# xiaohong-huang/RTK-Visual-Inertial-Navigation

Measured on AMD Instinct MI355X. Metric: gauss_newton_iterations_per_sec, higher is better.
Workload: dtype f64; 1 GPU; BASELINE cfg4: batch of 512 independent cfg3 windows (20 keyframes, 300 features, 3000 observations, 19 IMU factors, 10 satellites x 20 epochs carrier-phase+pseudorange, gauge prior) over the job, 8 dogleg iterations per solve; windows=512, windows_rank0=512

## Files before the change

### rtk_visual_inertial_navigation_amd/csrc/swf_dev.h

```cpp
#pragma once
#include <hip/hip_runtime.h>
#include <stdint.h>
#include "../../include/swf_types.h"

#define SWF_WAVE 64

struct WinRec {
    int x_base, x_n;
    int blk_base, n_blk;
    int loc_base, n_loc, n_e, n_red;
    long long S_base;
    long long Lt_base;
    int proj0, proj1;
    int lm0, lm1;
    int fr_base, nF;
    long long P_base;
    int gf0, gf1;
    int cl0, cl1;
    int pair0, pair1;
    int fsb0, fsb1;
    int tail_dim;
    int n_pose_blk;
    int lmb0, lmb1;
    int pch0, pch1;
// ... 36 lines not shown
    int j_off, r_off;
    int pad0, pad1;
};

struct Pair {
    int win;
    int ra, rb, la, lb;
    int fa, fb;
    int c0, c1;
    int is_diag;
    int loc_a;
    int fsb0, fsb1;
    int n, m;
    long long S_base, P_base;
    long long q_base;
};

struct AsmWin {
    int se0, ne;
    int ve0, nv;
    int n_red, m;
    int loc_base;
    int fs_base;
    int v_base;
    int win;
    long long C_base, S_base, P_base, q_base;
};
#define AS_NC(c) ((c) & 4095u)
#define AS_NP(c) (((c) >> 12) & 31u)
#define AS_NH(c) (((c) >> 17) & 4095u)
#define AS_DIAG(c) (((c) >> 29) & 1u)
#define AS_SOLD(c) (((c) >> 30) & 1u)

struct DevBatch {
    int n_win;
    int n_x, n_loc_total;
    int max_iter_trace;
    double* x; double* xc; double* x0;
    double* g; double* diag; double* rhs; double* y; double* step;
    double* vc;
    double* S; double* L;
    double* Wk;
    double* Linv;
    const WinRec* win; WinState* ws; swf_iteration* trace;
    const int* blk_xoff; const int* blk_loc; const int* blk_gs;
    const int* loc2x;
    const unsigned char* x_var;
    int n_proj;
    const int* p_win; const int* p_xpose; const int* p_xex; const int* p_xlm;
    const int* p_lpose; const int* p_llm; const int* p_fr; const int* p_lm;
    const double* p_uv;
    double* p_r; double* p_Jp; double* p_Jl;
    double* p_cpart; double* p_apart;
    int n_fsb; const int* fsb_win; const int* fsb_obs0; const int* fsb_perm; const int* fsb_foff; const int* fsb_foff0; const int* fsb_out0;
    double* fs_part;
    double* jsc;
    int n_lm;
    const int* lm_win; const int* lm_obs0; const int* lm_loc; const int* lm_col;
    double* lm_Einv; double* lm_g;
    double* P;
    double* lmq;
    const int* lmb_rec; int n_lmb;
    const int* sch_c0; const int* sch_rec;
    const int* sch_km;
    const unsigned long long* lm_fmask;
    int n_fr;
    const int* fr_obs0; const int* fr_obs;
    const int* fr_red;
    int n_gf;
    const GFac* gf;
    const int* s_x; const int* s_loc; const int* s_ls; const int* s_joff; const int* s_ccol;
    double* g_r; double* g_J; double* g_cost; double* g_aux;
    const double* imu_pre; const double* cp_dat; const double* pr_dat; const double* dop_dat; const double* sp_w;
    const double* gx_dat;
    int n_imu; const int* imu_gf;
    int n_idp; const int* idp_gf;
    int n_sc;  const int* sc_gf;
    int n_prior; const int* prior_gf;
    int n_pch; const int* pch_q; const int* pch_r0; const int* prior_nch;
    double* pr_cpart; double* pr_apart;
    const int* prior_dim; const long long* prior_Joff; const int* prior_roff; const int* prior_x0off;
    const double* prior_J; const double* prior_r0; const double* prior_x0;
    const double* prior_Jt;
    const int* prior_colloc;
    const int* prior_colcc;
    const int* s_pcol; const int* s_pxo;
    int n_cl;
    const Clique* cl;
    const int* cl_fac; const int* cl_frow;
    const int* cm_loc; const int* cm_ls; const int* cm_col;
    double* C; double* cv_graw; double* cv_dgraw; double* cv_cs; double* cE;
    const int* cv_loc;
    int n_clc[5]; const Clique* clc_rec[5];
    int n_cle; const Clique* cle_rec;
    int n_pair;
    const long long* pc_coff; const int* pc_cld; const int* pc_voff;
    int n_pd, n_po; const Pair* pair_d; const Pair* pair_o;
    const AsmWin* asw; int as_max_ne, as_max_nv;
    const int* as_dst; const unsigned* as_cnt; const int* as_src0; const int* as_aux; const int* as_src;
    const int* av_loc; const int* av_red; const unsigned* av_cnt; const int* av_src0; const int* av_i; const int* av_src;
    const unsigned* s_tnz;
    int spec;
    int rr_nmax;
};

__device__ __forceinline__ void qmul(const double* a, const double* b, double* o) {
    double ax = a[0], ay = a[1], az = a[2], aw = a[3];
// ... 247 lines not shown
```

### rtk_visual_inertial_navigation_amd/csrc/swf_engine.hip

```cpp
#include <hip/hip_runtime.h>
#include <algorithm>
#include <array>
#include <chrono>
#include <cmath>
#include <cstdio>
#include <cstdlib>
#include <cstring>
#include <map>
#include <string>
#include <memory>
#include <thread>
#include <vector>
#include "../../include/swf_solver.h"
#include "swf_kernels2.h"
#include "swf_kernels3.h"
#include "swf_kernels4.h"
#include "swf_lambda.h"

static thread_local std::string g_err;
static int fail(int code, const std::string& msg) { g_err = msg; return code; }
#define HIPCHK(x) do { hipError_t e_ = (x); if (e_ != hipSuccess) return fail(SWF_E_NODEVICE, std::string(#x) + ": " + hipGetErrorString(e_)); } while (0)

extern "C" const char* swf_last_error(void) { return g_err.c_str(); }
void swf_internal_set_error(const std::string& m) { g_err = m; }
// ... 868 lines not shown
                if (B.lm_loc[l] < 0) continue;
                int k = B.lm_obs0[l + 1] - B.lm_obs0[l];
                if (k > 64) { P.release(); delete b; return fail(SWF_E_UNSUPPORTED, "landmark with more than 64 observations"); }
                trs[(size_t)(l - W.lm0)] = tile_rows(B.lm_fmask[l]);
                ord.push_back(l);
            }
            auto key = [&](int l) { unsigned t = trs[(size_t)(l - W.lm0)]; int lo = t ? __builtin_ctz(t) : 0, hi = t ? 31 - __builtin_clz(t) : 0; return hi * 64 + lo; };
            std::stable_sort(ord.begin(), ord.end(), [&](int x, int y) { return key(x) < key(y); });
            const int first_task = (int)(rec.size() / 32);
            task_tiles.clear();
            size_t at = 0; int lw = 4;
            auto new_task = [&]() { at = rec.size(); rec.resize(at + 32, 0); for (int g = 0; g < 4; g++) rec[at + g * 8] = -1; task_tiles.emplace_back((size_t)ntl, 0u); lw = 0; };
            for (int l : ord) {
                int o0 = B.lm_obs0[l], k = B.lm_obs0[l + 1] - o0;
                if (lw >= 4) new_task();
                int* r = &rec[at + (size_t)lw * 8];
                r[0] = l; r[1] = B.lm_loc[l]; r[2] = o0; r[3] = o0 + k; r[4] = 3 * lw; r[5] = 0; r[6] = 0; r[7] = 0;
                unsigned t = trs[(size_t)(l - W.lm0)];
                const unsigned ks = lw == 0 ? 1u : lw == 1 ? 3u : lw == 2 ? 6u : 4u;
                std::vector<unsigned>& tt = task_tiles.back();
                for (int tr = 0; tr < nt; tr++) {
                    if (!((t >> tr) & 1u)) continue;
                    tt[(size_t)tr] |= ks;
                    for (int tc = 0; tc < tr; tc++) if ((t >> tc) & 1u) tt[(size_t)(nt + tr * (tr - 1) / 2 + tc)] |= ks;
                }
                lw++;
            }
            if (task_tiles.size() & 1) new_task();
            const int ntask = (int)task_tiles.size();
            for (int c = 0; c < ntask / TW; c++) {
                size_t kw = km.size(); km.resize(kw + (size_t)b->ls_kms, 0);
                for (int g = 0; g < TW; g++) {
                    const std::vector<unsigned>& tt = task_tiles[(size_t)(c * TW + g)];
                    for (int e = 0; e < ntl; e++) if (tt[(size_t)e]) {
                        b->lm_schur_mfma += __builtin_popcount(tt[(size_t)e]);
                        int lp = e / (NCW * TPW), r = e % (NCW * TPW), sl = r / NCW, cw = r % NCW;
                        km[kw + (size_t)(lp * NCW + cw)] |= (tt[(size_t)e] << (3 * g)) << (3 * TW * sl);
                    }
                }
            }
            const int np = ntask / 2;
            for (int sp = 0; sp < GEMM_SPLIT; sp++) c0.push_back(first_task + 2 * (int)((long long)sp * np / GEMM_SPLIT));
        }
        c0.push_back((int)(rec.size() / 32));
        rec.resize(rec.size() + (size_t)32 * 4 * LS_NB, 0);
        km.resize(km.size() + (size_t)b->ls_kms * 2, 0);
        PUT(sch_c0, c0); PUT(sch_rec, rec); PUT(sch_km, km);
    }
    D.n_fr = B.n_fr;
    B.fr_obs0.push_back((int)B.fr_obs.size());
    PUT(fr_obs0, B.fr_obs0); PUT(fr_obs, B.fr_obs); PUT(fr_red, B.fr_red);
    D.n_fsb = (int)B.fsb_win.size();
    B.fsb_obs0.push_back(D.n_proj); B.fsb_perm.resize((size_t)D.n_proj + 1, 0);
    PUT(fsb_win, B.fsb_win); PUT(fsb_obs0, B.fsb_obs0); PUT(fsb_perm, B.fsb_perm); PUT(fsb_foff, B.fsb_foff); PUT(fsb_foff0, B.fsb_foff0); PUT(fsb_out0, B.fsb_out0);
    rc |= P.zeros((size_t)B.fs_tot * FS_VAL, &D.fs_part);
    rc |= P.zeros((size_t)std::max<long long>(B.n_loc, 1), &D.jsc);
    D.n_gf = (int)B.gf.size();
    PUT(gf, B.gf);
    PUT(s_x, B.s_x); PUT(s_loc, B.s_loc); PUT(s_ls, B.s_ls); PUT(s_joff, B.s_joff); PUT(s_ccol, B.s_ccol);
    PUT(imu_pre, B.imu_pre); PUT(cp_dat, B.cp_dat); PUT(pr_dat, B.pr_dat); PUT(dop_dat, B.dop_dat); PUT(sp_w, B.sp_w); PUT(gx_dat, B.gx_dat);
    D.n_imu = (int)B.imu_gf.size(); D.n_sc = (int)B.sc_gf.size(); D.n_prior = (int)B.prior_gf.size();
    PUT(imu_gf, B.imu_gf); PUT(sc_gf, B.sc_gf); PUT(prior_gf, B.prior_gf); D.n_idp = (int)B.idp_gf.size(); PUT(idp_gf, B.idp_gf);
    PUT(prior_dim, B.prior_dim); PUT(prior_Joff, B.prior_Joff); PUT(prior_roff, B.prior_roff); PUT(prior_x0off, B.prior_x0off);
    {
        std::vector<double> Jt(B.prior_J.size());
        for (size_t k = 0; k < B.prior_dim.size(); k++) {
            const size_t n = (size_t)B.prior_dim[k]; const double* J = B.prior_J.data() + B.prior_Joff[k]; double* T = Jt.data() + B.prior_Joff[k];
            for (size_t r = 0; r < n; r++) for (size_t c = 0; c < n; c++) T[c * n + r] = J[r * n + c];
        }
        PUT(prior_Jt, Jt);
        std::vector<int> cl(B.prior_r0.size(), -1), cc(B.prior_r0.size(), -1), pcol(B.s_ls.size(), 0), pxo(B.s_ls.size(), 0);
        for (const GFac& G : B.gf) {
            if (G.type != GF_PRIOR) continue;
            int col = 0, xo = 0;
            for (int t = 0; t < G.nslot; t++) {
                int l = B.s_ls[G.slot0 + t], lo = B.s_loc[G.slot0 + t], mc = B.s_ccol[G.slot0 + t];
                pcol[G.slot0 + t] = col; pxo[G.slot0 + t] = xo;
                for (int q = 0; q < l; q++) {
                    cl[(size_t)B.prior_roff[G.data] + col + q] = lo >= 0 ? lo + q : -1;
                    cc[(size_t)B.prior_roff[G.data] + col + q] = mc >= 0 ? mc + q : -1;
                }
                col += l; xo += (l == 6 ? 7 : l);
            }
        }
        PUT(prior_colloc, cl); PUT(prior_colcc, cc); PUT(s_pcol, pcol); PUT(s_pxo, pxo);
    }
    PUT(prior_J, B.prior_J); PUT(prior_r0, B.prior_r0); PUT(prior_x0, B.prior_x0);
    D.n_cl = (int)B.cl.size();
    PUT(cl, B.cl); PUT(cl_fac, B.cl_fac); PUT(cl_frow, B.cl_frow); PUT(cm_loc, B.cm_loc); PUT(cm_ls, B.cm_ls); PUT(cm_col, B.cm_col);
    {
        std::vector<int> cvl((size_t)std::max(B.v_tot, 1), 0);
        for (const Clique& c : B.cl)
            for (int m = c.mem0; m < c.mem1; m++)
                for (int q = 0; q < B.cm_ls[(size_t)m]; q++) cvl[(size_t)c.v_off + (size_t)B.cm_col[(size_t)m] + (size_t)q] = B.cm_loc[(size_t)m] + q;
        PUT(cv_loc, cvl);
    }
    D.n_pair = (int)B.pair.size();
    PUT(pc_coff, B.pc_coff); PUT(pc_cld, B.pc_cld); PUT(pc_voff, B.pc_voff);
    {
        std::vector<int> pd, po, clc[5], cle;
        for (size_t i = 0; i < B.pair.size(); i++) {
            Pair& Pq = B.pair[i]; const WinRec& Rw = B.win[Pq.win];
            Pq.fsb0 = Rw.fsb0; Pq.fsb1 = Rw.fsb1; Pq.n = Rw.n_red; Pq.m = 6 * Rw.nF; Pq.S_base = Rw.S_base; Pq.P_base = Rw.P_base; Pq.q_base = (long long)6 * Rw.fr_base * GEMM_SPLIT;
            if (b->s_direct && !Pq.is_diag && Pq.fa >= 0 && Pq.fb >= 0 && Pq.c0 == Pq.c1) continue;
            (Pq.is_diag ? pd : po).push_back((int)i);
        }
        std::stable_sort(po.begin(), po.end(), [&](int a, int c) {
// ... 1118 lines not shown
    if (!ok) return fail(SWF_E_NODEVICE, "download failed");
    return SWF_OK;
}

#ifdef SWF_PROFILE_CHOL
extern "C" int swf_debug_chol_stamps(unsigned long long* out) {
    if (hipDeviceSynchronize() != hipSuccess) return SWF_E_NODEVICE;
    if (hipMemcpyFromSymbol(out, HIP_SYMBOL(g_chol_stamps), 64 * sizeof(unsigned long long)) != hipSuccess) return SWF_E_NODEVICE;
    return SWF_OK;
}
#endif

#ifdef SWF_PROFILE_CHOLW
extern "C" int swf_debug_chol_wstep(int step) {
    if (hipDeviceSynchronize() != hipSuccess) return SWF_E_NODEVICE;
    unsigned long long z[16 * 8] = { 0 };
    if (hipMemcpyToSymbol(HIP_SYMBOL(g_chol_wst), z, sizeof(z)) != hipSuccess) return SWF_E_NODEVICE;
    if (hipMemcpyToSymbol(HIP_SYMBOL(g_chol_wstep), &step, sizeof(int)) != hipSuccess) return SWF_E_NODEVICE;
    return SWF_OK;
}
extern "C" int swf_debug_chol_wstamps(unsigned long long* out) {
    if (hipDeviceSynchronize() != hipSuccess) return SWF_E_NODEVICE;
    if (hipMemcpyFromSymbol(out, HIP_SYMBOL(g_chol_wst), 16 * 8 * sizeof(unsigned long long)) != hipSuccess) return SWF_E_NODEVICE;
    return SWF_OK;
}
extern "C" int swf_debug_chol_pstamps(unsigned long long* out) {
    if (hipDeviceSynchronize() != hipSuccess) return SWF_E_NODEVICE;
    if (hipMemcpyFromSymbol(out, HIP_SYMBOL(g_chol_pst), 16 * sizeof(unsigned long long)) != hipSuccess) return SWF_E_NODEVICE;
    return SWF_OK;
}
extern "C" int swf_debug_chol_cstamps(unsigned long long* out) {
    if (hipDeviceSynchronize() != hipSuccess) return SWF_E_NODEVICE;
    if (hipMemcpyFromSymbol(out, HIP_SYMBOL(g_chol_cst), 32 * sizeof(unsigned long long)) != hipSuccess) return SWF_E_NODEVICE;
    return SWF_OK;
}
#endif

#ifdef SWF_PROFILE_DOG
extern "C" int swf_debug_dog_stamps(unsigned long long* out) {
    if (hipDeviceSynchronize() != hipSuccess) return SWF_E_NODEVICE;
    if (hipMemcpyFromSymbol(out, HIP_SYMBOL(g_dog_stamps), 16 * sizeof(unsigned long long)) != hipSuccess) return SWF_E_NODEVICE;
    return SWF_OK;
}
#endif

#ifdef SWF_PROFILE_CLQ
extern "C" int swf_debug_clq_stamps(unsigned long long* out) {
    if (hipDeviceSynchronize() != hipSuccess) return SWF_E_NODEVICE;
    if (hipMemcpyFromSymbol(out, HIP_SYMBOL(g_clq_stamps), 16 * sizeof(unsigned long long)) != hipSuccess) return SWF_E_NODEVICE;
    return SWF_OK;
}
#endif

#ifdef SWF_PROFILE_GEMM
extern "C" int swf_debug_gemm_stamps(unsigned long long* out) {
    if (hipDeviceSynchronize() != hipSuccess) return SWF_E_NODEVICE;
    if (hipMemcpyFromSymbol(out, HIP_SYMBOL(g_gemm_stamps), 16 * sizeof(unsigned long long)) != hipSuccess) return SWF_E_NODEVICE;
    return SWF_OK;
}
#endif


struct swf_composite {
    CompArgs A{};
    std::vector<void*> bufs;
    int n = 0, nmax = 0, nmin = 0; long long sumM = 0, sumN = 0, sumG = 0, sumG2 = 0;
    std::vector<int> M;
    bool eigen_root = false;
    hipStream_t stream = nullptr;
    ~swf_composite() { for (void* p : bufs) (void)hipFree(p); }
};

extern "C" int swf_composite_destroy(swf_composite* c) { delete c; return SWF_OK; }

extern "C" int swf_composite_create(int32_t n, const int32_t* M, const int32_t* N, const double* pose, const double* sb,
                                    const double* pose_lin, const double* sb_lin, const double* Hpp, const double* HpN,
                                    const double* rhs_p, const double* HNN, const double* rhsN, const double* pre,
                                    const double pbg[3], const double gw[3], void* stream, swf_composite** out) {
    if (!out || n <= 0 || !M || !N || !pose || !sb || !pose_lin || !sb_lin || !Hpp || !HpN || !rhs_p || !HNN || !rhsN || !pre || !pbg || !gw)
        return fail(SWF_E_INVALID, "swf_composite_create: null argument");
    std::vector<int> eo(n + 1, 0), no(n + 1, 0);
    std::vector<long long> pno(n + 1, 0), nno(n + 1, 0), go(n + 1, 0), g2o(n + 1, 0);
    int nmax_ = 0, nmin_ = 1 << 30;
    for (int f = 0; f < n; f++) {
        if (M[f] < 1) return fail(SWF_E_INVALID, "composite factor without hidden epochs");
        if (N[f] < 0 || N[f] > CO_MAXN) return fail(SWF_E_UNSUPPORTED, "composite factor with more than 64 ambiguities");
        nmax_ = std::max(nmax_, (int)N[f]); nmin_ = std::min(nmin_, (int)N[f]);
        eo[f + 1] = eo[f] + M[f]; no[f + 1] = no[f] + N[f];
        pno[f + 1] = pno[f] + 15LL * M[f] * N[f]; nno[f + 1] = nno[f] + (long long)N[f] * N[f];
        go[f + 1] = go[f] + 30 + N[f]; g2o[f + 1] = g2o[f] + (long long)(30 + N[f]) * (30 + N[f]);
    }
    std::unique_ptr<swf_composite> c(new swf_composite());
    c->n = n; c->nmax = nmax_; c->nmin = nmin_; c->sumM = eo[n]; c->sumN = no[n]; c->sumG = go[n]; c->sumG2 = g2o[n]; c->stream = (hipStream_t)stream;
    bool bad = false;
    auto up = [&](const void* src, size_t bytes) -> void* {
        void* d = nullptr;
        if (hipMalloc(&d, std::max<size_t>(bytes, 8)) != hipSuccess) { bad = true; return nullptr; }
        c->bufs.push_back(d);
        if (src) { if (hipMemcpy(d, src, bytes, hipMemcpyHostToDevice) != hipSuccess) bad = true; }
        else if (hipMemset(d, 0, std::max<size_t>(bytes, 8)) != hipSuccess) bad = true;
        return d;
    };
    CompArgs& A = c->A;
    const size_t D = sizeof(double);
    A.n = n;
    A.M = (const int*)up(M, n * sizeof(int)); A.N = (const int*)up(N, n * sizeof(int));
// ... 86 lines not shown
```

### rtk_visual_inertial_navigation_amd/csrc/swf_kernels.h

```cpp
#pragma once
#include "swf_dev.h"

struct DevOpt {
    int max_iter, step_mode, strategy, jacobi;
    double r0, max_r, min_r, min_rel_dec, ftol, gtol, ptol, min_mu, max_mu, mu_inc, min_diag, max_diag;
};



__device__ __forceinline__ double damp_diag(const DevOpt& O, double d, double* jsc_slot, bool first) {
    if (!O.jacobi) return clampd(d, O.min_diag, O.max_diag);
    double q;
    if (first) { double r = 1.0 + sqrt(d > 0.0 ? d : 0.0); q = r * r; *jsc_slot = q; }
    else q = *jsc_slot;
    return clampd(d / q, O.min_diag, O.max_diag) * q;
}

template <bool JAC> __device__ __forceinline__ bool eval_gate(const DevBatch& B, const WinState& s) { return B.spec == 2 ? true : (JAC && !B.spec) ? s.need_lin != 0 : s.eval_cand != 0; }
template <bool JAC> __device__ __forceinline__ const double* eval_src(const DevBatch& B) { return (JAC && !B.spec) ? B.x : B.xc; }

#define CLIGHT_D 299792458.0
#define OMGE_D 7.2921151467E-5

template <bool JAC, bool STORE>
__device__ __forceinline__ double proj_core(const DevBatch& B, int i, const WinRec& W, const double* P, const double* E, const double* X,
                                          double u0, double u1, bool jp, bool jl, double* keep);
template <bool JAC, bool STORE = true>
__device__ __forceinline__ double d_eval_proj_at(const DevBatch& B, int i, double* keep) {
    int w = B.p_win[i];
    const WinState& s = B.ws[w];
    if (!eval_gate<JAC>(B, s)) return 0.0;
    const WinRec& W = B.win[w];
    const double* xs = eval_src<JAC>(B);
    const double* pose = xs + B.p_xpose[i];
    const double* ex = xs + B.p_xex[i];
    const double* lm = xs + B.p_xlm[i];
    double P[7], E[7], X[3];
#pragma unroll
    for (int k = 0; k < 7; k++) { P[k] = pose[k]; E[k] = ex[k]; }
    X[0] = lm[0]; X[1] = lm[1]; X[2] = lm[2];
    return proj_core<JAC, STORE>(B, i, W, P, E, X, B.p_uv[2 * i], B.p_uv[2 * i + 1], JAC && B.p_lpose[i] >= 0, JAC && B.p_llm[i] >= 0, keep);
}
template <bool JAC, bool STORE>
__device__ __forceinline__ double proj_core(const DevBatch& B, int i, const WinRec& W, const double* P, const double* E, const double* X,
                                          double u0, double u1, bool jp, bool jl, double* keep) {
    double Qj_inv[4], qic_inv[4], d[3], pts_imu[3], t[3], pc[3];
    qinv(P + 3, Qj_inv);
    qinv(E + 3, qic_inv);
    d[0] = X[0] - P[0]; d[1] = X[1] - P[1]; d[2] = X[2] - P[2];
    qrot(Qj_inv, d, pts_imu);
    t[0] = pts_imu[0] + W.pbg[0] - E[0]; t[1] = pts_imu[1] + W.pbg[1] - E[1]; t[2] = pts_imu[2] + W.pbg[2] - E[2];
    qrot(qic_inv, t, pc);
    double dep = pc[2], si = W.proj_sqrt_info;
    double r0 = si * (pc[0] / dep - u0);
    double r1 = si * (pc[1] / dep - u1);
    double sr = 1.0, cost;
    double sq = r0 * r0 + r1 * r1;
    if (W.proj_loss_a > 0) {
        double b = W.proj_loss_a * W.proj_loss_a, c = 1.0 / b;
        double sum = 1.0 + sq * c, inv = 1.0 / sum;
        cost = 0.5 * b * log(sum);
        sr = sqrt(inv > 2.2250738585072014e-308 ? inv : 2.2250738585072014e-308);
    } else cost = 0.5 * sq;
    if (!JAC) return cost;
    int n = B.n_proj;
    if (STORE) { B.p_r[i] = r0 * sr; B.p_r[n + i] = r1 * sr; }
    if (keep) { keep[12] = r0 * sr; keep[13] = r1 * sr; }
    if (!jp && !jl) return cost;
    double Rj[9], ric[9], ricT[9], RjT[9], A[9];
    q2R(P + 3, Rj); q2R(E + 3, ric);
    mat3T(ric, ricT); mat3T(Rj, RjT);
    double red[6] = { si * (1. / dep), 0, si * (-pc[0] / (dep * dep)), 0, si * (1. / dep), si * (-pc[1] / (dep * dep)) };
    mat3mul(ricT, RjT, A);
    if (jp) {
        double S[9], Bm[9];
        skew3(pts_imu, S);
        mat3mul(ricT, S, Bm);
#pragma unroll
        for (int a = 0; a < 2; a++)
#pragma unroll
            for (int j = 0; j < 3; j++) {
                double u = 0, v = 0;
#pragma unroll
                for (int k = 0; k < 3; k++) { u += red[a * 3 + k] * -A[k * 3 + j]; v += red[a * 3 + k] * Bm[k * 3 + j]; }
                if (STORE) { if (!jl) B.p_Jp[(a * 6 + j) * n + i] = u * sr; B.p_Jp[(a * 6 + 3 + j) * n + i] = v * sr; }
                if (keep) { keep[a * 6 + j] = u * sr; keep[a * 6 + 3 + j] = v * sr; }
            }
    }
    if (jl) {
#pragma unroll
        for (int a = 0; a < 2; a++)
#pragma unroll
            for (int j = 0; j < 3; j++) {
                double u = 0;
#pragma unroll
                for (int k = 0; k < 3; k++) u += red[a * 3 + k] * A[k * 3 + j];
                if (STORE) B.p_Jl[(a * 3 + j) * n + i] = u * sr;
                if (keep) keep[14 + a * 3 + j] = u * sr;
            }
    }
    return cost;
}

__device__ __forceinline__ void d_eval_proj_cost(const DevBatch& B, int blk) {
    __shared__ double csum[16];
    const int w = B.fsb_win[blk];
    if (!eval_gate<false>(B, B.ws[w])) return;
    const int o_beg = B.fsb_obs0[blk], cnt = B.fsb_obs0[blk + 1] - o_beg, tid = threadIdx.x;
    double c = 0.0;
    if (tid < cnt) c = d_eval_proj_at<false>(B, o_beg + tid, nullptr);
    c = block_sum(c, csum);
    if (tid == 0) B.p_cpart[blk] = c;
}

__device__ __forceinline__ void imu_unwhitened(const double* pi, const double* sbi, const double* pj, const double* sbj,
                               const double* pre, const double* pbg, const double* gw,
                               double* raw, double* U, bool jac, int part) {
    const double* Pi = pi; const double* Qi = pi + 3;
    const double* Vi = sbi; const double* Bai = sbi + 3; const double* Bgi = sbi + 6;
    const double* Pj = pj; const double* Qj = pj + 3;
    const double* Vj = sbj; const double* Baj = sbj + 3; const double* Bgj = sbj + 6;
    const double* dp = pre + SWF_PRE_DP; const double* dq = pre + SWF_PRE_DQ; const double* dv = pre + SWF_PRE_DV;
    const double* lba = pre + SWF_PRE_LBA; const double* lbg = pre + SWF_PRE_LBG;
    const double* dp_dba = pre + SWF_PRE_DP_DBA; const double* dp_dbg = pre + SWF_PRE_DP_DBG;
    const double* dq_dbg = pre + SWF_PRE_DQ_DBG; const double* dv_dba = pre + SWF_PRE_DV_DBA;
    const double* dv_dbg = pre + SWF_PRE_DV_DBG;
    double T = pre[SWF_PRE_SUMDT];
    const double* gyri = pre + SWF_PRE_GYRI; const double* gyrj = pre + SWF_PRE_GYRJ;
    double Qi_inv[4];
    qinv(Qi, Qi_inv);
#define SETU(R0, C0, MAT, SGN) for (int i_ = 0; i_ < 3; i_++) for (int j_ = 0; j_ < 3; j_++) U[(R0 + i_) * 30 + C0 + j_] = SGN * MAT[i_ * 3 + j_];
    if (part == 0 || part == 2) {
        double dbg[3], th[3], dqc[4], cq[4], cq_inv[4], wj[3], wjPbg[3];
        for (int k = 0; k < 3; k++) { dbg[k] = Bgi[k] - lbg[k]; wj[k] = gyrj[k] - Bgj[k]; }
        mat3vec(dq_dbg, dbg, th);
        dqc[0] = th[0] / 2; dqc[1] = th[1] / 2; dqc[2] = th[2] / 2; dqc[3] = 1.0;
        qmul(dq, dqc, cq);
        cross3(wj, pbg, wjPbg);
        qinv(cq, cq_inv);
        if (part == 0) {
            double dba[3], cv[3], cp[3], t1[3], t2[3], QjPbg[3], wi[3], wiPbg[3], QjwjPbg[3];
            for (int k = 0; k < 3; k++) { dba[k] = Bai[k] - lba[k]; wi[k] = gyri[k] - Bgi[k]; }
            mat3vec(dv_dba, dba, t1); mat3vec(dv_dbg, dbg, t2);
            for (int k = 0; k < 3; k++) cv[k] = dv[k] + t1[k] + t2[k];
            mat3vec(dp_dba, dba, t1); mat3vec(dp_dbg, dbg, t2);
            for (int k = 0; k < 3; k++) cp[k] = dp[k] + t1[k] + t2[k];
            qrot(Qj, pbg, QjPbg);
            cross3(wi, pbg, wiPbg);
            qrot(Qj, wjPbg, QjwjPbg);
            double ap[3], av[3], rp[3], rv[3];
            for (int k = 0; k < 3; k++) {
                ap[k] = 0.5 * gw[k] * T * T + ((Pj[k] - Pi[k]) - QjPbg[k]) - Vi[k] * T;
                av[k] = gw[k] * T + (Vj[k] - QjwjPbg[k]) - Vi[k];
            }
            qrot(Qi_inv, ap, rp);
            qrot(Qi_inv, av, rv);
            for (int k = 0; k < 3; k++) {
                raw[0 + k] = rp[k] - cp[k] + pbg[k] + wiPbg[k] * T;
                raw[6 + k] = rv[k] - cv[k] + wiPbg[k];
                raw[9 + k] = Baj[k] - Bai[k];
                raw[12 + k] = Bgj[k] - Bgi[k];
            }
            double qij[4], e[4];
// ... 980 lines not shown
    } else {
        for (int j = tid; j < df; j += CB_NT) B.cv_cs[C.v_off + j] = 0.0;
    }
    const long long ntri = (long long)df * (df + 1) / 2;
    for (long long t = tid; t < ntri; t += CB_NT) {
        int i = (int)((sqrt(8.0 * (double)t + 1.0) - 1.0) * 0.5);
        while ((long long)(i + 1) * (i + 2) / 2 <= t) i++;
        while ((long long)i * (i + 1) / 2 > t) i--;
        int j = (int)(t - (long long)i * (i + 1) / 2);
        const double* ci = Jc + (size_t)(de + i) * ldj; const double* cj = Jc + (size_t)(de + j) * ldj;
        double m = 0;
#pragma unroll 4
        for (int k = 0; k < nrow; k++) m += ci[k] * cj[k];
        for (int a = 0; a < de; a++) m -= Me[a * d + de + i] * Tt[a * df + j];
        Cm[(size_t)i * df + j] = m; Cm[(size_t)j * df + i] = m;
    }
}
#undef bad_s
__global__ void __launch_bounds__(CB_NT) k_clique_big(DevBatch B, DevOpt O) {
    __shared__ double Me[CB_MAXED];
    __shared__ double Tt[CB_MAXED];
    __shared__ double Ei[9][9];
    __shared__ double Eg[9], ge[9];
    __shared__ int bad_sv;
    __shared__ double Jl[CB_LDS_J];
    if ((int)blockIdx.x >= B.n_clc[3]) return;
    const Clique& C = B.clc_rec[3][blockIdx.x];
    if ((long long)(C.n_rows | 1) * (C.d_e + C.d_f) <= CB_LDS_J) d_clique_big<true>(B, O, Me, Tt, Ei, Eg, ge, &bad_sv, Jl);
    else d_clique_big<false>(B, O, Me, Tt, Ei, Eg, ge, &bad_sv, Jl);
}
#define CB_LDS_J2 11008
__global__ void __launch_bounds__(CB_NT) k_clique_big2(DevBatch B, DevOpt O) {
    if ((int)blockIdx.x >= B.n_clc[3]) {
        static_assert(CB_NT >= 256, "k_clique_big2: the clique rows keep the four waves d_clique_elim<..., NW = 4> synchronises");
        if (threadIdx.x >= 256) return;
        d_clique_elim<64, 64, 9, 2, 8, 4, 4>(B, O, (int)blockIdx.x - B.n_clc[3]);
        return;
    }
    __shared__ double Me[CB_MAXED];
    __shared__ double Tt[CB_MAXED];
    __shared__ double Ei[9][9];
    __shared__ double Eg[9], ge[9];
    __shared__ int bad_sv;
    __shared__ double Jl[CB_LDS_J2];
    const Clique& C = B.clc_rec[3][blockIdx.x];
    if ((long long)(C.n_rows | 1) * (C.d_e + C.d_f) <= CB_LDS_J2) d_clique_big<true>(B, O, Me, Tt, Ei, Eg, ge, &bad_sv, Jl);
    else d_clique_big<false>(B, O, Me, Tt, Ei, Eg, ge, &bad_sv, Jl);
}

#define FS_BLK 256
#define FS_VAL 27
#define FS_HALF 14
__device__ __forceinline__ void d_eval_proj_fs(const DevBatch& B, int blk, double (*V)[FS_HALF], int* foff) {
    int w = B.fsb_win[blk];
    if (!eval_gate<true>(B, B.ws[w])) return;
    const WinRec& W = B.win[w];
    int o_beg = B.fsb_obs0[blk], cnt = B.fsb_obs0[blk + 1] - o_beg, tid = threadIdx.x;
    int nF = W.nF;
    for (int e = tid; e <= nF; e += FS_BLK) foff[e] = B.fsb_foff[B.fsb_foff0[blk] + e];
    double keep[20];
#pragma unroll
    for (int k = 0; k < 20; k++) keep[k] = 0.0;
    int rk = 0;
    double cost = 0.0;
    if (tid < cnt) { rk = B.fsb_perm[o_beg + tid]; cost = d_eval_proj_at<true>(B, o_beg + tid, keep); }
    {
        __shared__ double csum[16];
        cost = block_sum(cost, csum);
        if (tid == 0) B.p_cpart[blk] = cost;
    }
    double val[FS_VAL];
    {
        const double* a = keep; const double* b = keep + 6;
        int k = 0;
#pragma unroll
        for (int i = 0; i < 6; i++)
#pragma unroll
            for (int j = 0; j <= i; j++) val[k++] = a[i] * a[j] + b[i] * b[j];
#pragma unroll
        for (int i = 0; i < 6; i++) val[21 + i] = a[i] * keep[12] + b[i] * keep[13];
    }
    double* out = B.fs_part + (size_t)B.fsb_out0[blk] * FS_VAL;
#pragma unroll
    for (int half = 0; half < 2; half++) {
        const int v0 = half * FS_HALF, nv = half == 0 ? FS_HALF : FS_VAL - FS_HALF;
        if (half) __syncthreads();
        if (tid < cnt) {
#pragma unroll
            for (int k = 0; k < FS_HALF; k++) if (k < nv) V[rk][k] = val[v0 + k];
        }
        __syncthreads();
        for (int e = tid; e < nF * nv; e += FS_BLK) {
            int f = e / nv, v = e - f * nv;
            double acc = 0;
            int q = foff[f], q1 = foff[f + 1];
            for (; q + 4 <= q1; q += 4) {
                double x0 = V[q][v], x1 = V[q + 1][v], x2 = V[q + 2][v], x3 = V[q + 3][v];
                acc += x0; acc += x1; acc += x2; acc += x3;
            }
            for (; q < q1; q++) acc += V[q][v];
            out[f * FS_VAL + v0 + v] = acc;
        }
    }
}

__device__ __forceinline__ double as_sum(const double* base, const int* src, int n, int add = 0) {
    double v = 0;
    int c = 0;
    for (; c + 4 <= n; c += 4) {
        const int i0 = src[c], i1 = src[c + 1], i2 = src[c + 2], i3 = src[c + 3];
        const double x0 = base[i0 + add], x1 = base[i1 + add], x2 = base[i2 + add], x3 = base[i3 + add];
        v += x0; v += x1; v += x2; v += x3;
    }
    for (; c < n; c++) v += base[src[c] + add];
    return v;
}
__global__ void __launch_bounds__(256) k_assemble_flat(DevBatch B, DevOpt O, int write_S, int nbS) {
    const AsmWin& A = B.asw[blockIdx.y];
    const WinState& s = B.ws[A.win];
    if (!s.need_lin) return;
    const int tid = threadIdx.x;
    if ((int)blockIdx.x < nbS) {
        if (!write_S) return;
        const int e = blockIdx.x * 256 + tid;
        if (e >= A.ne) return;
        const int k = A.se0 + e;
        const unsigned cnt = B.as_cnt[k];
        const int nC = AS_NC(cnt), nP = AS_NP(cnt), nH = AS_NH(cnt);
        const int* src = B.as_src + B.as_src0[k];
        const int dst = B.as_dst[k];
        double* S = B.S + A.S_base;
        const double* C = B.C + A.C_base;
        const double sold = AS_SOLD(cnt) ? S[dst] : 0.0;
        double v = as_sum(C, src, nC);
        if (AS_SOLD(cnt)) v = sold + v;
        else if (nP) v -= as_sum(B.P + A.P_base, src + nC, nP);
        double hs = 0;
        if (nH) { hs = as_sum(B.fs_part + (size_t)A.fs_base * FS_VAL, src + nC + nP, nH); v += hs; }
        if (AS_DIAG(cnt)) {
            const double* dgr = B.cv_dgraw + A.v_base;
            const int* sd = src + nC + nP + nH;
            double dg = hs;
            int c = 0;
            for (; c + 4 <= nC; c += 4) { const double x0 = dgr[sd[c]], x1 = dgr[sd[c + 1]], x2 = dgr[sd[c + 2]], x3 = dgr[sd[c + 3]]; dg += x0; dg += x1; dg += x2; dg += x3; }
            for (; c < nC; c++) dg += dgr[sd[c]];
            v += s.mu * damp_diag(O, dg, B.jsc + A.loc_base + B.as_aux[k], s.iter == 0);
        }
        S[dst] = v;
        return;
    }
    const int e = (blockIdx.x - nbS) * 256 + tid;
    if (e >= A.nv) return;
    const int k = A.ve0 + e;
    const unsigned cnt = B.av_cnt[k];
    const int nC = AS_NC(cnt), nQ = AS_NP(cnt), nH = AS_NH(cnt);
    const int* src = B.av_src + B.av_src0[k];
// ... 23 lines not shown
```

### rtk_visual_inertial_navigation_amd/csrc/swf_kernels2.h

```cpp
#pragma once
#include "swf_kernels.h"

#define CH_NB 32
#ifndef CH_OCC
#define CH_OCC 2
#endif
#ifndef CH_KU
#define CH_KU 4
#endif
__device__ __forceinline__ double row_newbcast_d(double v, int n) {
    int lo = __double2loint(v), hi = __double2hiint(v);
    switch (n) {
#define NB_CASE(K) case K: lo = __builtin_amdgcn_mov_dpp(lo, 0x150 + K, 0xf, 0xf, false); hi = __builtin_amdgcn_mov_dpp(hi, 0x150 + K, 0xf, 0xf, false); break;
        NB_CASE(0) NB_CASE(1) NB_CASE(2) NB_CASE(3) NB_CASE(4) NB_CASE(5) NB_CASE(6) NB_CASE(7)
        NB_CASE(8) NB_CASE(9) NB_CASE(10) NB_CASE(11) NB_CASE(12) NB_CASE(13) NB_CASE(14) NB_CASE(15)
#undef NB_CASE
    }
    return __hiloint2double(hi, lo);
}
__device__ __forceinline__ double bperm_d(double v, int idx_bytes) {
    int lo = __builtin_amdgcn_ds_bpermute(idx_bytes, __double2loint(v));
    int hi = __builtin_amdgcn_ds_bpermute(idx_bytes, __double2hiint(v));
    return __hiloint2double(hi, lo);
}
// ... 726 lines not shown
        aux = a0 * a0 + a1 * a1;
        if (pfr >= 0) { c0 = -(jl0 * w0 + jl3 * w1); c1 = -(jl1 * w0 + jl4 * w1); c2 = -(jl2 * w0 + jl5 * w1); }
    }
    (void)n;
    sc[0][tid] = c0; sc[1][tid] = c1; sc[2][tid] = c2;
    {
        __shared__ double asum[16];
        aux = block_sum(aux, asum);
        if (tid == 0) B.p_apart[bid] = aux;
    }
    if (!hl || failed || lloc < 0) return;
    double t0 = 0, t1 = 0, t2 = 0;
    for (int q = lob - o0, qe = loe - o0; q < qe; q++) { t0 += sc[0][q]; t1 += sc[1][q]; t2 += sc[2][q]; }
    t0 += g0; t1 += g1; t2 += g2;
    B.y[lloc] = e00 * t0 + e10 * t1 + e20 * t2;
    B.y[lloc + 1] = e10 * t0 + e11 * t1 + e21 * t2;
    B.y[lloc + 2] = e20 * t0 + e21 * t1 + e22 * t2;
}
__device__ __forceinline__ void d_backsub_clique(const DevBatch& B, int bid) {
    int q = (bid * blockDim.x + threadIdx.x) >> 4, sub = threadIdx.x & 15, lane = threadIdx.x & 63;
    bool valid = q < B.n_cle;
    const Clique& C = B.cle_rec[valid ? q : B.n_cle - 1];
    const WinState& s = B.ws[C.win];
    bool act = valid && s.need_lin && !s.lin_fail;
    int de = C.d_e, df = C.d_f;
    const double* E = B.cE + C.e_off;
    const double* M = E + de * de;
    double part[9];
#pragma unroll
    for (int a = 0; a < 9; a++) part[a] = 0;
    const int* cl = B.cv_loc + C.v_off;
    for (int c = sub; c < (act ? df : 0); c += 16) {
        const double yv = B.y[cl[c]];
#pragma unroll
        for (int a = 0; a < 9; a++) if (a < de) part[a] += M[a * df + c] * yv;
    }
    double t = 0;
#pragma unroll
    for (int a = 0; a < 9; a++) { double pa = grp16_sum(part[a]); if (sub == a) t = pa; }
    if (act && sub < de) t = M[de * df + sub] - t;
    double acc = 0;
#pragma unroll
    for (int b = 0; b < 9; b++) {
        double tb = __shfl(t, (lane & ~15) + b, 64);
        if (act && sub < de && b < de) acc += E[sub * de + b] * tb;
    }
    if (act && sub < de) B.y[C.e_loc + sub] = acc;
}


struct Segs { int e[8]; };

template <bool JAC, bool FS = false, bool IMU = false>
__global__ void __launch_bounds__(256) k_eval_ps(DevBatch B, Segs S) {
    constexpr int SM_PRIOR = 2 * PRIOR_LDS_DIM + 16, SM_FS = FS ? FS_BLK * FS_HALF + 168 / 2 + 1 : 1;
    __shared__ double sm[SM_PRIOR > SM_FS ? SM_PRIOR : SM_FS];
    int bid = blockIdx.x;
    if (bid < S.e[0]) { static_assert(FS && JAC, "the projection segment evaluates Jacobians by frame-sum block"); d_eval_proj_fs(B, bid, (double (*)[FS_HALF])sm, (int*)(sm + FS_BLK * FS_HALF)); }
    else if (bid < S.e[1]) d_eval_scalar<JAC>(B, bid - S.e[0]);
    else if (!IMU || bid < S.e[2]) d_eval_prior<JAC>(B, bid - S.e[1], sm);
    else d_eval_imu<JAC>(B, bid - S.e[2]);
}
template <int PART>
__global__ void __launch_bounds__(256) k_post_chol(DevBatch B, DevOpt O, Segs S) {
    int bid = blockIdx.x + (PART == 2 ? S.e[0] : 0);
    __shared__ double sm_bs[PART == 2 ? 1 : 3][256];
    __shared__ double sm_pv[PART == 1 ? 1 : PRB_MAX]; __shared__ int sm_pl[PART == 1 ? 1 : PRB_MAX]; __shared__ double sm_pw[4];
    if (PART != 2 && bid < S.e[0]) { d_backsub_lm(B, O, bid, sm_bs); return; }
    if (PART == 1) return;
    if (bid < S.e[1]) d_backsub_clique(B, bid - S.e[0]);
    else if (bid < S.e[3]) d_jtimes_scalar<0>(B, O, bid - S.e[2]);
    else if (bid < S.e[4]) d_jtimes_imu<0>(B, O, bid - S.e[3]);
    else d_jtimes_prior<0>(B, O, bid - S.e[4], sm_pv, sm_pl, sm_pw);
}
template <bool WITH_IMU, int PART>
__global__ void __launch_bounds__(256) k_post_dogleg(DevBatch B, DevOpt O, Segs S) {
    __shared__ double sm_prior[PART == 1 ? 1 : 2 * PRIOR_LDS_DIM + 16];
    int bid = blockIdx.x;
    if (PART == 1) { d_eval_proj_cost(B, bid); return; }
    if (PART == 2) bid += S.e[0];
    if (PART == 0 && bid < S.e[0]) d_eval_proj_cost(B, bid);
    else if (bid < S.e[1]) d_eval_scalar<false>(B, bid - S.e[0]);
    else if (bid < S.e[2]) d_eval_prior<false>(B, bid - S.e[1], sm_prior);
    else if (WITH_IMU) d_eval_imu<false>(B, bid - S.e[2]);
}

#define WP_LDS 256
__device__ __forceinline__ void win_part_stage(const double* part, int q0, int q1, double* st) {
    for (int q = q0 + (int)threadIdx.x; q < q1 && q - q0 < WP_LDS; q += (int)blockDim.x) st[q - q0] = part[q];
}
__device__ __forceinline__ double win_part_sum(const double* part, int q0, int q1, const double* st) {
    double a = 0;
    const int n = q1 - q0;
    for (int q = 0; q < n && q < WP_LDS; q++) a += st[q];
    for (int q = WP_LDS; q < n; q++) a += part[q0 + q];
    return a;
}
__device__ __forceinline__ double win_cost_sum(const DevBatch& B, const WinRec& W, double* red, double* st ) {
    win_part_stage(B.p_cpart, W.fsb0, W.fsb1, st);
    win_part_stage(B.pr_cpart, W.pch0, W.pch1, st + WP_LDS);
    double a = 0;
    for (int i = W.gf0 + threadIdx.x; i < W.gf1; i += blockDim.x) a += B.g_cost[i];
    a = block_sum(a, red);
    return (win_part_sum(B.p_cpart, W.fsb0, W.fsb1, st) + win_part_sum(B.pr_cpart, W.pch0, W.pch1, st + WP_LDS)) + a;
}
__device__ __forceinline__ double win_x_norm(const DevBatch& B, const WinRec& W, const double* x, double* red) {
    double a = 0;
// ... 473 lines not shown
```

Baseline: 663,900 iterations/s.

## Pack frame-sum block metadata into records and hoist projection loads ahead of gating

Replaces the separate per-block arrays (window, obs start, foff0, out0) with one packed 8-int record per frame-sum block, read as two int4 loads that also carry the observation count and frame count. The per-observation loads (indices, uv, state vector, perm rank, frame offsets) are all issued up front in a ProjBlk loader before the gate check, which shortens the chain of dependent memory loads. It also adds a minimum-occupancy launch bound on the projection eval kernel and optional timing stamps behind a profile macro. In exchange, blocks that end up gated off still issue their speculative loads, and the occupancy hint may force register spills.

Result: faster. 677,200 iterations/s (median of 6 runs) (+2.0%).

```diff
diff --git a/rtk_visual_inertial_navigation_amd/csrc/swf_dev.h b/rtk_visual_inertial_navigation_amd/csrc/swf_dev.h
--- a/rtk_visual_inertial_navigation_amd/csrc/swf_dev.h
+++ b/rtk_visual_inertial_navigation_amd/csrc/swf_dev.h
@@ -112,7 +112,7 @@
     const double* p_uv;
     double* p_r; double* p_Jp; double* p_Jl;
     double* p_cpart; double* p_apart;
-    int n_fsb; const int* fsb_win; const int* fsb_obs0; const int* fsb_perm; const int* fsb_foff; const int* fsb_foff0; const int* fsb_out0;
+    int n_fsb; const int* fsb_rec; const int* fsb_perm; const int* fsb_foff;
     double* fs_part;
     double* jsc;
     int n_lm;
diff --git a/rtk_visual_inertial_navigation_amd/csrc/swf_engine.hip b/rtk_visual_inertial_navigation_amd/csrc/swf_engine.hip
--- a/rtk_visual_inertial_navigation_amd/csrc/swf_engine.hip
+++ b/rtk_visual_inertial_navigation_amd/csrc/swf_engine.hip
@@ -944,7 +944,16 @@
     PUT(fr_obs0, B.fr_obs0); PUT(fr_obs, B.fr_obs); PUT(fr_red, B.fr_red);
     D.n_fsb = (int)B.fsb_win.size();
     B.fsb_obs0.push_back(D.n_proj); B.fsb_perm.resize((size_t)D.n_proj + 1, 0);
-    PUT(fsb_win, B.fsb_win); PUT(fsb_obs0, B.fsb_obs0); PUT(fsb_perm, B.fsb_perm); PUT(fsb_foff, B.fsb_foff); PUT(fsb_foff0, B.fsb_foff0); PUT(fsb_out0, B.fsb_out0);
+    {
+        std::vector<int> rec((size_t)8 * std::max(D.n_fsb, 1), 0);
+        for (int k = 0; k < D.n_fsb; k++) {
+            int* r = rec.data() + (size_t)8 * k;
+            r[0] = B.fsb_win[(size_t)k]; r[1] = B.fsb_obs0[(size_t)k]; r[2] = B.fsb_obs0[(size_t)k + 1] - B.fsb_obs0[(size_t)k];
+            r[3] = B.fsb_foff0[(size_t)k]; r[4] = B.fsb_out0[(size_t)k]; r[5] = B.win[(size_t)r[0]].nF;
+        }
+        PUT(fsb_rec, rec);
+    }
+    PUT(fsb_perm, B.fsb_perm); PUT(fsb_foff, B.fsb_foff);
     rc |= P.zeros((size_t)B.fs_tot * FS_VAL, &D.fs_part);
     rc |= P.zeros((size_t)std::max<long long>(B.n_loc, 1), &D.jsc);
     D.n_gf = (int)B.gf.size();
@@ -2169,6 +2178,14 @@
 }
 #endif
 
+#ifdef SWF_PROFILE_EVAL
+extern "C" int swf_debug_eval_stamps(unsigned long long* out) {
+    if (hipDeviceSynchronize() != hipSuccess) return SWF_E_NODEVICE;
+    if (hipMemcpyFromSymbol(out, HIP_SYMBOL(g_eval_stamps), 16 * sizeof(unsigned long long)) != hipSuccess) return SWF_E_NODEVICE;
+    return SWF_OK;
+}
+#endif
+
 #ifdef SWF_PROFILE_GEMM
 extern "C" int swf_debug_gemm_stamps(unsigned long long* out) {
     if (hipDeviceSynchronize() != hipSuccess) return SWF_E_NODEVICE;
diff --git a/rtk_visual_inertial_navigation_amd/csrc/swf_kernels.h b/rtk_visual_inertial_navigation_amd/csrc/swf_kernels.h
--- a/rtk_visual_inertial_navigation_amd/csrc/swf_kernels.h
+++ b/rtk_visual_inertial_navigation_amd/csrc/swf_kernels.h
@@ -25,22 +25,49 @@
 template <bool JAC, bool STORE>
 __device__ __forceinline__ double proj_core(const DevBatch& B, int i, const WinRec& W, const double* P, const double* E, const double* X,
                                           double u0, double u1, bool jp, bool jl, double* keep);
-template <bool JAC, bool STORE = true>
-__device__ __forceinline__ double d_eval_proj_at(const DevBatch& B, int i, double* keep) {
-    int w = B.p_win[i];
-    const WinState& s = B.ws[w];
-    if (!eval_gate<JAC>(B, s)) return 0.0;
-    const WinRec& W = B.win[w];
-    const double* xs = eval_src<JAC>(B);
-    const double* pose = xs + B.p_xpose[i];
-    const double* ex = xs + B.p_xex[i];
-    const double* lm = xs + B.p_xlm[i];
-    double P[7], E[7], X[3];
-#pragma unroll
-    for (int k = 0; k < 7; k++) { P[k] = pose[k]; E[k] = ex[k]; }
-    X[0] = lm[0]; X[1] = lm[1]; X[2] = lm[2];
-    return proj_core<JAC, STORE>(B, i, W, P, E, X, B.p_uv[2 * i], B.p_uv[2 * i + 1], JAC && B.p_lpose[i] >= 0, JAC && B.p_llm[i] >= 0, keep);
-}
+#ifdef SWF_PROFILE_EVAL
+__device__ unsigned long long g_eval_stamps[16];
+#define EST(i) do { if (blockIdx.x == 0 && threadIdx.x == 0) { __builtin_amdgcn_s_waitcnt(0); unsigned long long t_ = __builtin_amdgcn_s_memtime(); g_eval_stamps[i] = t_ - te_; te_ = t_; } } while (0)
+#else
+#define EST(i)
+#endif
+template <bool JAC>
+struct ProjBlk {
+    int cnt, foff0, out0, nF, rk, lp, ll, fo;
+    bool gate;
+    WinRec W;
+    double P[7], E[7], X[3], u0, u1;
+    int o;
+#ifdef SWF_PROFILE_EVAL
+    unsigned long long te_;
+#endif
+    __device__ __forceinline__ void load(const DevBatch& B, int blk) {
+#ifdef SWF_PROFILE_EVAL
+        te_ = __builtin_amdgcn_s_memtime();
+#endif
+        const int4 r0 = ((const int4*)B.fsb_rec)[2 * blk], r1 = ((const int4*)B.fsb_rec)[2 * blk + 1];
+        const int w = r0.x, tid = threadIdx.x;
+        cnt = r0.z; foff0 = r0.w; out0 = r1.x; nF = r1.y;
+        o = tid < cnt ? r0.y + tid : r0.y;
+        if (JAC) EST(0);
+        const WinState& s = B.ws[w];
+        const WinRec& Wg = B.win[w];
+        const int need = s.need_lin, cand = s.eval_cand;
+        W.pbg[0] = Wg.pbg[0]; W.pbg[1] = Wg.pbg[1]; W.pbg[2] = Wg.pbg[2]; W.proj_sqrt_info = Wg.proj_sqrt_info; W.proj_loss_a = Wg.proj_loss_a;
+        const int xpo = B.p_xpose[o], xex = B.p_xex[o], xlm = B.p_xlm[o];
+        lp = JAC ? B.p_lpose[o] : -1; ll = JAC ? B.p_llm[o] : -1; rk = JAC ? B.fsb_perm[o] : 0;
+        u0 = B.p_uv[2 * o]; u1 = B.p_uv[2 * o + 1];
+        fo = JAC ? B.fsb_foff[foff0 + (tid <= nF ? tid : 0)] : 0;
+        if (JAC) EST(1);
+        const double* xs = eval_src<JAC>(B);
+#pragma unroll
+        for (int k = 0; k < 7; k++) { P[k] = xs[xpo + k]; E[k] = xs[xex + k]; }
+#pragma unroll
+        for (int k = 0; k < 3; k++) X[k] = xs[xlm + k];
+        if (JAC) EST(2);
+        gate = B.spec == 2 ? true : (JAC && !B.spec) ? need != 0 : cand != 0;
+    }
+};
 template <bool JAC, bool STORE>
 __device__ __forceinline__ double proj_core(const DevBatch& B, int i, const WinRec& W, const double* P, const double* E, const double* X,
                                           double u0, double u1, bool jp, bool jl, double* keep) {
@@ -102,13 +129,23 @@
     return cost;
 }
 
+template <bool JAC>
+__device__ __forceinline__ double d_eval_proj_at(const DevBatch& B, const ProjBlk<JAC>& Q, double* keep) {
+    double P[7], E[7], X[3];
+#pragma unroll
+    for (int k = 0; k < 7; k++) { P[k] = Q.P[k]; E[k] = Q.E[k]; }
+    X[0] = Q.X[0]; X[1] = Q.X[1]; X[2] = Q.X[2];
+    return proj_core<JAC, true>(B, Q.o, Q.W, P, E, X, Q.u0, Q.u1, JAC && Q.lp >= 0, JAC && Q.ll >= 0, keep);
+}
+
 __device__ __forceinline__ void d_eval_proj_cost(const DevBatch& B, int blk) {
     __shared__ double csum[16];
-    const int w = B.fsb_win[blk];
-    if (!eval_gate<false>(B, B.ws[w])) return;
-    const int o_beg = B.fsb_obs0[blk], cnt = B.fsb_obs0[blk + 1] - o_beg, tid = threadIdx.x;
+    ProjBlk<false> Q;
+    Q.load(B, blk);
+    if (!Q.gate) return;
+    const int tid = threadIdx.x;
     double c = 0.0;
-    if (tid < cnt) c = d_eval_proj_at<false>(B, o_beg + tid, nullptr);
+    if (tid < Q.cnt) c = d_eval_proj_at<false>(B, Q, nullptr);
     c = block_sum(c, csum);
     if (tid == 0) B.p_cpart[blk] = c;
 }
@@ -1195,23 +1232,27 @@
 #define FS_VAL 27
 #define FS_HALF 14
 __device__ __forceinline__ void d_eval_proj_fs(const DevBatch& B, int blk, double (*V)[FS_HALF], int* foff) {
-    int w = B.fsb_win[blk];
-    if (!eval_gate<true>(B, B.ws[w])) return;
-    const WinRec& W = B.win[w];
-    int o_beg = B.fsb_obs0[blk], cnt = B.fsb_obs0[blk + 1] - o_beg, tid = threadIdx.x;
-    int nF = W.nF;
-    for (int e = tid; e <= nF; e += FS_BLK) foff[e] = B.fsb_foff[B.fsb_foff0[blk] + e];
+    ProjBlk<true> Q;
+    Q.load(B, blk);
+#ifdef SWF_PROFILE_EVAL
+    unsigned long long& te_ = Q.te_;
+#endif
+    const int tid = threadIdx.x, cnt = Q.cnt, nF = Q.nF, rk = Q.rk;
+    if (!Q.gate) return;
+    if (tid <= nF) foff[tid] = Q.fo;
+    for (int e = tid + FS_BLK; e <= nF; e += FS_BLK) foff[e] = B.fsb_foff[Q.foff0 + e];
     double keep[20];
 #pragma unroll
     for (int k = 0; k < 20; k++) keep[k] = 0.0;
-    int rk = 0;
     double cost = 0.0;
-    if (tid < cnt) { rk = B.fsb_perm[o_beg + tid]; cost = d_eval_proj_at<true>(B, o_beg + tid, keep); }
+    if (tid < cnt) cost = d_eval_proj_at<true>(B, Q, keep);
+    EST(3);
     {
         __shared__ double csum[16];
         cost = block_sum(cost, csum);
         if (tid == 0) B.p_cpart[blk] = cost;
     }
+    EST(4);
     double val[FS_VAL];
     {
         const double* a = keep; const double* b = keep + 6;
@@ -1223,7 +1264,7 @@
 #pragma unroll
         for (int i = 0; i < 6; i++) val[21 + i] = a[i] * keep[12] + b[i] * keep[13];
     }
-    double* out = B.fs_part + (size_t)B.fsb_out0[blk] * FS_VAL;
+    double* out = B.fs_part + (size_t)Q.out0 * FS_VAL;
 #pragma unroll
     for (int half = 0; half < 2; half++) {
         const int v0 = half * FS_HALF, nv = half == 0 ? FS_HALF : FS_VAL - FS_HALF;
@@ -1245,6 +1286,7 @@
             out[f * FS_VAL + v0 + v] = acc;
         }
     }
+    EST(5);
 }
 
 __device__ __forceinline__ double as_sum(const double* base, const int* src, int n, int add = 0) {
diff --git a/rtk_visual_inertial_navigation_amd/csrc/swf_kernels2.h b/rtk_visual_inertial_navigation_amd/csrc/swf_kernels2.h
--- a/rtk_visual_inertial_navigation_amd/csrc/swf_kernels2.h
+++ b/rtk_visual_inertial_navigation_amd/csrc/swf_kernels2.h
@@ -802,7 +802,7 @@
 struct Segs { int e[8]; };
 
 template <bool JAC, bool FS = false, bool IMU = false>
-__global__ void __launch_bounds__(256) k_eval_ps(DevBatch B, Segs S) {
+__global__ void __launch_bounds__(256, (FS && !IMU) ? 5 : 1) k_eval_ps(DevBatch B, Segs S) {
     constexpr int SM_PRIOR = 2 * PRIOR_LDS_DIM + 16, SM_FS = FS ? FS_BLK * FS_HALF + 168 / 2 + 1 : 1;
     __shared__ double sm[SM_PRIOR > SM_FS ? SM_PRIOR : SM_FS];
     int bid = blockIdx.x;
```
